# aikiriao/SLA

Hardware: AMD Instinct MI355X
Metric: encode Msamples/s (LPC+residual path), verified bit-exact vs the oracle in this run (higher is better)
Workload: dtype f64+int32

## Files before the change

### sla_amd/csrc/kernels/expand.inc

```
#define EXPAND_THREADS 1024
typedef uint32_t ex_u32x4 __attribute__((ext_vector_type(4), aligned(4)));
typedef uint32_t ex_u32x2 __attribute__((ext_vector_type(2), aligned(4)));
#define EXPAND_PER 8
#define EXPAND_TILE (EXPAND_THREADS * EXPAND_PER)
#define EXPAND_MAX_WINDOWS 256
#define EXPAND_MAX_LEN 16384u
__device__ __forceinline__ uint32_t expand_window(const uint32_t* s_wlen, const uint32_t* s_woff, uint32_t num_win, uint32_t len)
{
  for (uint32_t q = 0; q < num_win; q++) { if (s_wlen[q] == len) { return s_woff[q]; } }
  return SLA_HIP_NO_WINDOW;
}

__device__ __forceinline__ bool expand_range_is_zero(const uint64_t* __restrict__ nz, uint32_t from, uint32_t count)
{
  uint64_t pos = from;
  const uint64_t end = (uint64_t)from + count;
  while (pos < end) {
    const uint64_t word = nz[pos >> 6] >> (pos & 63u);
    if (word != 0ull) { pos += (uint64_t)__builtin_ctzll(word); break; }
    pos += 64u - (pos & 63u);
  }
  return pos >= end;
}

__global__ __launch_bounds__(EXPAND_THREADS)
void k_expand_scan(const sla_hip_superframe* __restrict__ sf, uint32_t num_sf, const uint32_t* __restrict__ parts,
                   const uint32_t* __restrict__ nparts, const uint32_t* __restrict__ status, uint32_t nch,
                   const uint32_t* __restrict__ win_len, uint32_t num_win,
                   uint32_t* __restrict__ run, uint32_t* __restrict__ prefix, uint32_t capacity,
                   volatile uint32_t* counts, uint32_t sequence, const uint64_t* __restrict__ nz)
{
  __shared__ uint32_t s_has[EXPAND_MAX_LEN / 32 + 1];
  __shared__ uint32_t s_cb[EXPAND_TILE], s_cl[EXPAND_TILE];
  __shared__ uint32_t s_wb[EXPAND_THREADS / 64], s_wl[EXPAND_THREADS / 64];
  __shared__ uint32_t s_bad;
  const uint32_t t = threadIdx.x, lane = t & 63, wv = t >> 6;
  if (t == 0) { s_bad = (run[2] != 0u || num_win > EXPAND_MAX_WINDOWS) ? 1u : 0u; }
  for (uint32_t i = t; i < EXPAND_MAX_LEN / 32 + 1; i += EXPAND_THREADS) { s_has[i] = 0u; }
  __syncthreads();
  for (uint32_t i = t; i < num_win && i < EXPAND_MAX_WINDOWS; i += EXPAND_THREADS) {
    const uint32_t len = win_len[i];
    if (len != 0u && len <= EXPAND_MAX_LEN) { atomicOr(&s_has[len >> 5], 1u << (len & 31u)); }
  }
  const uint32_t run_b = run[0], run_g = run[1];
  uint32_t base_b = 0, base_l = 0;
  bool bad = false;
  __syncthreads();
  for (uint32_t t0 = 0; t0 < num_sf; t0 += EXPAND_TILE) {
    uint32_t live[EXPAND_PER], np[EXPAND_PER], st[EXPAND_PER], len0[EXPAND_PER];
#pragma unroll
    for (int k = 0; k < EXPAND_PER; k++) {
      const uint32_t i = t0 + (uint32_t)k * EXPAND_THREADS + t;
      live[k] = (i < num_sf) ? sf[i].live : SLA_HIP_NOT_LIVE;
    }
#pragma unroll
    for (int k = 0; k < EXPAND_PER; k++) {
      const bool l = (live[k] != SLA_HIP_NOT_LIVE);
      np[k] = l ? nparts[live[k]] : 0u;
      st[k] = l ? status[live[k]] : 0u;
      len0[k] = l ? parts[(uint64_t)live[k] * PLAN_NODES] : 0u;
    }
#pragma unroll
    for (int k = 0; k < EXPAND_PER; k++) {
      const uint32_t i = t0 + (uint32_t)k * EXPAND_THREADS + t;
      const bool l = (live[k] != SLA_HIP_NOT_LIVE);
      if (l && (st[k] != 0u || np[k] == 0u || np[k] > PLAN_NODES)) { bad = true; np[k] = 0; }
      uint32_t quiet = 0u, at = (l && nz != nullptr) ? sf[i].start : 0u;
      for (uint32_t p = 0; l && p < np[k]; p++) {
        const uint32_t len = (p == 0) ? len0[k] : parts[(uint64_t)live[k] * PLAN_NODES + p];
        if (len == 0u || len > EXPAND_MAX_LEN || ((s_has[len >> 5] >> (len & 31u)) & 1u) == 0u) { bad = true; }
        else if (nz != nullptr) { if (expand_range_is_zero(nz, at, len)) { quiet++; } at += len; }
      }
      s_cb[(uint32_t)k * EXPAND_THREADS + t] = (i < num_sf) ? (l ? np[k] : 1u) : 0u;
      s_cl[(uint32_t)k * EXPAND_THREADS + t] = l ? np[k] - quiet : 0u;
    }
    __syncthreads();
    uint32_t cb[EXPAND_PER], cl[EXPAND_PER], my_b = 0, my_l = 0;
#pragma unroll
    for (int k = 0; k < EXPAND_PER; k++) { cb[k] = s_cb[t * EXPAND_PER + k]; cl[k] = s_cl[t * EXPAND_PER + k]; my_b += cb[k]; my_l += cl[k]; }
    uint32_t inc_b = my_b, inc_l = my_l;
#pragma unroll
    for (int off = 1; off < 64; off <<= 1) {
      const uint32_t ob = (uint32_t)__shfl_up((int)inc_b, off), ol = (uint32_t)__shfl_up((int)inc_l, off);
      if (lane >= (uint32_t)off) { inc_b += ob; inc_l += ol; }
    }
    if (lane == 63) { s_wb[wv] = inc_b; s_wl[wv] = inc_l; }
    __syncthreads();
    uint32_t off_b = run_b + base_b + (inc_b - my_b), off_l = base_l + (inc_l - my_l), tile_b = 0, tile_l = 0;
    for (uint32_t w = 0; w < EXPAND_THREADS / 64; w++) {
      const uint32_t vb = s_wb[w], vl = s_wl[w];
      if (w < wv) { off_b += vb; off_l += vl; }
      tile_b += vb; tile_l += vl;
    }
#pragma unroll
    for (int k = 0; k < EXPAND_PER; k++) {
      const uint32_t i = t0 + t * EXPAND_PER + (uint32_t)k;
      if (i < num_sf) { ex_u32x2 w; w.x = off_b; w.y = off_l; *reinterpret_cast<ex_u32x2*>(prefix + 2 * (uint64_t)i) = w; }
      off_b += cb[k]; off_l += cl[k];
    }
    base_b += tile_b; base_l += tile_l;
    __syncthreads();
  }
  if (bad) { s_bad = 1u; }
  __syncthreads();
  if (t == 0) {
    const bool ok = (s_bad == 0u) && ((uint64_t)run_g + (uint64_t)base_l * nch <= (uint64_t)capacity);
    run[3] = run_g;
    if (ok) { run[0] = run_b + base_b; run[1] = run_g + base_l * nch; } else { run[2] = 1u; }
    counts[0] = ok ? base_b : 0u; counts[1] = ok ? base_l * nch : 0u; counts[2] = ok ? 1u : 0u;
    __threadfence_system();
    counts[3] = sequence;
    __threadfence_system();
  }
}

__global__ __launch_bounds__(256)
void k_expand_write(const sla_hip_superframe* __restrict__ sf, uint32_t num_sf, const uint32_t* __restrict__ parts,
                    const uint32_t* __restrict__ nparts, uint32_t nch, uint32_t int_shift,
                    const uint32_t* __restrict__ win_len, const uint32_t* __restrict__ win_off, uint32_t num_win,
                    const uint32_t* __restrict__ run, const uint32_t* __restrict__ prefix,
                    sla_hip_lpc_group* __restrict__ groups, sla_hip_lpc_cand* __restrict__ cands, sla_hip_acf_job* __restrict__ acf_jobs,
                    const uint64_t* __restrict__ nz)
{
  __shared__ uint32_t s_wlen[EXPAND_MAX_WINDOWS], s_woff[EXPAND_MAX_WINDOWS];
  if (run[2] != 0u) { return; }
  for (uint32_t i = threadIdx.x; i < num_win && i < EXPAND_MAX_WINDOWS; i += blockDim.x) { s_wlen[i] = win_len[i]; s_woff[i] = win_off[i]; }
  __syncthreads();
  const uint32_t i = blockIdx.x * blockDim.x + threadIdx.x;
  if (i >= num_sf) { return; }
  const sla_hip_superframe f = sf[i];
  if (f.live == SLA_HIP_NOT_LIVE) { return; }
  const uint32_t run_g = run[3];
  const uint32_t np = nparts[f.live];
  uint32_t b = prefix[2 * (uint64_t)i], l = prefix[2 * (uint64_t)i + 1], at = f.start;
  for (uint32_t p = 0; p < np; p++, b++) {
    const uint32_t len = parts[(uint64_t)f.live * PLAN_NODES + p];
    if (nz != nullptr && expand_range_is_zero(nz, at, len)) { at += len; continue; }
    const uint32_t woff = expand_window(s_wlen, s_woff, num_win, len);
    for (uint32_t ch = 0; ch < nch; ch++) {
      const uint32_t g = run_g + l * nch + ch;
      static_assert(sizeof(sla_hip_lpc_group) == 40 && sizeof(sla_hip_lpc_cand) == 8 && sizeof(sla_hip_acf_job) == 16, "descriptor layout");
      ex_u32x4 w0, w1; ex_u32x2 w2, wc; ex_u32x4 wa;
      w0.x = at; w0.y = 0u; w0.z = len; w0.w = ch;
      w1.x = woff; w1.y = int_shift; w1.z = g; w1.w = 1u;
      w2.x = b * nch + ch; w2.y = 0u;
      uint32_t* gp = reinterpret_cast<uint32_t*>(groups + g);
      *reinterpret_cast<ex_u32x4*>(gp) = w0; *reinterpret_cast<ex_u32x4*>(gp + 4) = w1; *reinterpret_cast<ex_u32x2*>(gp + 8) = w2;
      wc.x = 0u; wc.y = len;
      *reinterpret_cast<ex_u32x2*>(cands + g) = wc;
      wa.x = at; wa.y = 0u; wa.z = len; wa.w = ch;
      *reinterpret_cast<ex_u32x4*>(acf_jobs + g) = wa;
    }
    at += len; l++;
  }
}
```

### sla_amd/csrc/kernels/launchers.inc

```
static inline unsigned long long* span_of(const sla_hip_launch_extra* x) { return (x != nullptr) ? x->d_span : nullptr; }

static thread_local sla_hip_tuning t_tuning_val;
static thread_local bool t_tuning_set = false;
extern "C" void sla_hip_use_tuning(const sla_hip_tuning* tuning)
{
  if (tuning != nullptr) { t_tuning_val = *tuning; t_tuning_set = true; } else { t_tuning_set = false; }
}
static inline sla_hip_tuning tuning()
{
  sla_hip_tuning t;
  memset(&t, 0, sizeof(t));
  if (t_tuning_set) { t = t_tuning_val; }
  if (!(t.plan_margin >= PLAN_MARGIN)) { t.plan_margin = 0.0; }
  return t;
}

static hipError_t ensure_dynamic_lds(const void* fn, size_t bytes)
{
  static struct { const void* fn; int dev; size_t bytes; } seen[64];
  static int nseen = 0;
  static pthread_mutex_t mu = PTHREAD_MUTEX_INITIALIZER;
  int dev = 0;
  (void)hipGetDevice(&dev);
  pthread_mutex_lock(&mu);
// ... 411 lines not shown
extern "C" int sla_hip_launch_expand_masked(const sla_hip_superframe* d_superframes, uint32_t num_superframes,
                                     const uint32_t* d_parts, const uint32_t* d_num_parts, const uint32_t* d_status,
                                     uint32_t num_channels, uint32_t int_shift,
                                     const uint32_t* d_win_len, const uint32_t* d_win_off, uint32_t num_windows,
                                     uint32_t* d_run, uint32_t* d_prefix, sla_hip_lpc_group* d_groups, sla_hip_lpc_cand* d_cands,
                                     sla_hip_acf_job* d_acf_jobs, uint32_t group_capacity,
                                     uint32_t* counts, uint32_t sequence, const uint64_t* d_nonzero_mask, sla_hip_stream_t stream);

extern "C" int sla_hip_launch_expand(const sla_hip_superframe* d_superframes, uint32_t num_superframes,
                                     const uint32_t* d_parts, const uint32_t* d_num_parts, const uint32_t* d_status,
                                     uint32_t num_channels, uint32_t int_shift,
                                     const uint32_t* d_win_len, const uint32_t* d_win_off, uint32_t num_windows,
                                     uint32_t* d_run, uint32_t* d_prefix, sla_hip_lpc_group* d_groups, sla_hip_lpc_cand* d_cands,
                                     sla_hip_acf_job* d_acf_jobs, uint32_t group_capacity,
                                     uint32_t* counts, uint32_t sequence, sla_hip_stream_t stream)
{
  return sla_hip_launch_expand_masked(d_superframes, num_superframes, d_parts, d_num_parts, d_status, num_channels, int_shift, d_win_len,
                                      d_win_off, num_windows, d_run, d_prefix, d_groups, d_cands, d_acf_jobs, group_capacity, counts, sequence,
                                      nullptr, stream);
}

extern "C" int sla_hip_launch_expand_masked(const sla_hip_superframe* d_superframes, uint32_t num_superframes,
                                     const uint32_t* d_parts, const uint32_t* d_num_parts, const uint32_t* d_status,
                                     uint32_t num_channels, uint32_t int_shift,
                                     const uint32_t* d_win_len, const uint32_t* d_win_off, uint32_t num_windows,
                                     uint32_t* d_run, uint32_t* d_prefix, sla_hip_lpc_group* d_groups, sla_hip_lpc_cand* d_cands,
                                     sla_hip_acf_job* d_acf_jobs, uint32_t group_capacity,
                                     uint32_t* counts, uint32_t sequence, const uint64_t* d_nonzero_mask, sla_hip_stream_t stream)
{
  if (d_superframes == nullptr || d_parts == nullptr || d_num_parts == nullptr || d_status == nullptr || d_run == nullptr
      || d_prefix == nullptr || d_groups == nullptr || d_cands == nullptr || d_acf_jobs == nullptr || counts == nullptr
      || (num_windows != 0 && (d_win_len == nullptr || d_win_off == nullptr))) { return SLA_APIRESULT_INVALID_ARGUMENT; }
  if (num_channels == 0 || num_channels > 8 || int_shift > 31) { return SLA_APIRESULT_INVALID_ARGUMENT; }
  hipLaunchKernelGGL(k_expand_scan, dim3(1), dim3(EXPAND_THREADS), 0, (hipStream_t)stream, d_superframes, num_superframes, d_parts,
                     d_num_parts, d_status, num_channels, d_win_len, num_windows, d_run, d_prefix, group_capacity,
                     (volatile uint32_t*)counts, sequence, d_nonzero_mask);
  if (num_superframes != 0) {
    hipLaunchKernelGGL(k_expand_write, dim3((num_superframes + 255) / 256), dim3(256), 0, (hipStream_t)stream, d_superframes, num_superframes,
                       d_parts, d_num_parts, num_channels, int_shift, d_win_len, d_win_off, num_windows, d_run, d_prefix, d_groups, d_cands,
                       d_acf_jobs, d_nonzero_mask);
  }
  return hip_rc(hipGetLastError());
}

extern "C" int sla_hip_launch_lattice(const int32_t* d_pcm, uint64_t plane_stride, uint32_t mid_side, uint32_t order,
                                      const sla_hip_lattice_chunk* d_chunks, uint32_t num_chunks,
                                      const int32_t* d_kint, int32_t* d_residual, sla_hip_stream_t stream)
{
  if (d_pcm == nullptr || d_chunks == nullptr || d_kint == nullptr || d_residual == nullptr) { return SLA_APIRESULT_INVALID_ARGUMENT; }
  if (order < 1 || order > 255 || (order + LAT_T - 1) / LAT_T >= 32) { return SLA_APIRESULT_INVALID_ARGUMENT; }
  if (num_chunks == 0) { return 0; }
  hipLaunchKernelGGL(k_lattice, dim3((num_chunks + 3) / 4), dim3(256), 0, (hipStream_t)stream, d_pcm, plane_stride,
                     mid_side, order, d_chunks, num_chunks, d_kint, d_residual, (unsigned long long*)nullptr, tuning().lattice_plain ? 2u : 0u);
  return hip_rc(hipGetLastError());
}

extern "C" int sla_hip_launch_lattice_groups_x(const int32_t* d_pcm, uint64_t plane_stride, uint32_t mid_side, uint32_t order,
                                             const sla_hip_lpc_group* d_groups, uint32_t num_groups, uint32_t max_window,
                                             const int32_t* d_kint, int32_t* d_residual, sla_hip_stream_t stream, const sla_hip_launch_extra* extra)
{
  if (d_pcm == nullptr || d_groups == nullptr || d_kint == nullptr || d_residual == nullptr) { return SLA_APIRESULT_INVALID_ARGUMENT; }
  if (order < 1 || order > 255 || (order + LAT_T - 1) / LAT_T >= 32 || max_window == 0) { return SLA_APIRESULT_INVALID_ARGUMENT; }
  if (num_groups == 0) { return 0; }
  const uint32_t per = (SLA_WAVE - (order + LAT_T - 1) / LAT_T) * LAT_T;
  const uint32_t cpg = (max_window + per - 1) / per;
  const uint64_t waves = (uint64_t)num_groups * cpg;
  if (waves > 0x7FFFFFFFull) { return SLA_APIRESULT_EXCEED_HANDLE_CAPACITY; }
  hipLaunchKernelGGL(k_lattice_groups, dim3((uint32_t)((waves + 3) / 4)), dim3(256), 0, (hipStream_t)stream, d_pcm, plane_stride,
                     mid_side, order, d_groups, num_groups, cpg, d_kint, d_residual, span_of(extra), tuning().lattice_plain ? 2u : 0u);
// ... 277 lines not shown
```

### sla_amd/csrc/sla_encoder.c

```c
#define _GNU_SOURCE
#include "sla_internal.h"
#include "SLADecoder.h"

#include <math.h>
#include <pthread.h>
#include <sched.h>
#include <stdio.h>
#include <stdlib.h>
#include <string.h>
#include <time.h>
#include <unistd.h>

#define STATUS_WAVE_FORMAT   (1u << 0)
#define STATUS_ENCODE_PARAM  (1u << 1)
#define MAX_ANALYSIS_WINDOW  16384u

typedef struct { void* ptr; size_t cap; } devbuf_t;
typedef struct { void* ptr; size_t cap; } pinbuf_t;
typedef struct { void* ptr; size_t cap; } hostbuf_t;

typedef struct {
  uint32_t start, nsmpl, type, bytes;
} blk_t;

// ... 44 lines not shown
  int      device_expand;
  int      expand_silence;
  uint32_t silence_runs;
  devbuf_t d_zruns, d_zscratch; pinbuf_t h_zruns;
  slai_silence sil;
  uint32_t sil_stat[4];
  uint32_t expand_seq;
  uint32_t expanded_chunks;
  int      table_cache, tab_valid;
  uint32_t tab_key[10], tab_cnt[12];
  void*    tab_sf; void* tab_shapes;
  uint32_t winmap_entries;
  uint32_t table_hits;
  int      spec_valid; uint32_t spec_or;
  uint32_t spec_misses;
  uint32_t blocks_exact;
  sla_hip_tuning tune;
  uint32_t host_planned;
  uint32_t fallback_groups;
  uint32_t tail_launches;
  slai_fft_plan* fft;
  uint32_t threads;
  struct slai_pool* pool;

  devbuf_t d_pcm, d_res1, d_res2, d_or, d_nz, d_groups, d_cands, d_lpc_out, d_code, d_kint, d_rshift,
           d_winpool, d_chunks, d_jobs, d_fold, d_acf_jobs, d_acf, d_acf_scratch, d_twiddle, d_bgroups, d_bcands, d_blk_out, d_kk, d_pk_jobs, d_pk_blocks, d_pk_hdr, d_image,
           d_xgroups, d_tile_sums, d_fgroups, d_parts, d_nparts, d_pstatus, d_spans, d_cert_flag, d_fb_list, d_fb_count,
           d_sframes, d_winmap, d_run, d_expref, d_fast_twiddle, d_ltm_eps, d_ltm_list;
  int twiddle_ready;
  pinbuf_t h_nz, h_groups, h_cands, h_lpc_out, h_code, h_kint, h_rshift, h_chunks, h_jobs, h_fold, h_res, h_pcm, h_acf_jobs, h_acf,
           h_bgroups, h_bcands, h_blk_out, h_pk_jobs, h_pk_blocks, h_pk_hdr, h_xgroups, h_fgroups, h_parts, h_nparts, h_pstatus, h_cert_flag,
           h_sframes, h_winmap, h_counts;
  devbuf_t d_rice; pinbuf_t h_rice;
  hostbuf_t w_job_blk, w_job_ch, w_job_grp, w_grp_of_slot, w_parts, w_nparts, w_status;
  uint32_t* h_or;
  size_t nz_ones_cap; uint64_t nz_ones_words;
  pinbuf_t h_stage[2]; devbuf_t d_stage[2]; hipEvent_t ev_stage[2];
  hipEvent_t ev_prep;
  int      groups_valid;
  hipEvent_t ev_pack[4];

  double*   win_host; size_t win_count, win_cap;
  uint32_t* win_len; uint32_t* win_off; uint32_t win_entries, win_entries_cap;
  SLAWindowFunctionType win_type; int win_dirty;

  int32_t* user_res1; int32_t* user_res2; uint64_t user_stride;

  uint32_t file_or_word;
  int      skip_prepass;

  uint32_t nsegs; const uint32_t* seg_start; const uint32_t* seg_len;
  uint32_t batch_lshift, batch_or;
  devbuf_t d_tile_or; pinbuf_t h_tile_or;
  devbuf_t d_binfo; pinbuf_t h_binfo;
  devbuf_t d_ingest; pinbuf_t h_ingest;
  hipEvent_t ev_order;
  int      batch_silence;
  int      mask_absent;
  uint32_t* tab_segs; uint32_t tab_nsegs;

  int      stream_mode;
  uint32_t stream_piece;
  uint32_t stream_lanes;
  uint32_t batch_lanes;
  pthread_mutex_t* upload_gate;
  double   batch_stamp[4];
// ... 1630 lines not shown
  for (j = 0; j < a->njobs; j++) {
    if (e->device_ltm) {
      const sla_hip_tail_job* jb = (const sla_hip_tail_job*)e->h_jobs.ptr + j;
      blkch_t* bc = &e->bc[(size_t)a->job_blk[j] * C + a->job_ch[j]];
      uint32_t t;
      if (e->blk[a->job_blk[j]].type != SLAI_BLK_COMPRESS) { continue; }
      bc->pitch = jb->pitch;
      for (t = 0; t < SLAI_MAX_TAPS; t++) { bc->ltm_q[t] = jb->ltm_coef[t]; }
    }
    {
    const uint64_t mean = fold[j] / e->blk[a->job_blk[j]].nsmpl;
    const uint32_t init = (uint32_t)(mean > 1 ? mean : 1);
    const uint32_t kept = (uint32_t)((((uint64_t)(uint32_t)(init << 8)) + 128u) >> 8);
    e->bc[(size_t)a->job_blk[j] * C + a->job_ch[j]].rice_init = kept ? kept : 1u;
    }
  }
}

typedef struct { struct SLAEncoder* e; const actx_t* a; } home_ctx_t;

static void jobs_home_one(void* vctx, uint32_t j)
{
  const home_ctx_t* c = (const home_ctx_t*)vctx;
  struct SLAEncoder* e = c->e;
  const uint32_t b = c->a->job_blk[j];
  const sla_hip_tail_job* jb = (const sla_hip_tail_job*)e->h_jobs.ptr + j;
  blkch_t* bc = &e->bc[(size_t)b * e->wave_format.num_channels + c->a->job_ch[j]];
  uint32_t t;
  if (e->blk[b].type != SLAI_BLK_COMPRESS) { return; }
  bc->pitch = jb->pitch;
  for (t = 0; t < SLAI_MAX_TAPS; t++) { bc->ltm_q[t] = jb->ltm_coef[t]; }
}

static void rice_home_one(void* vctx, uint32_t j)
{
  const home_ctx_t* c = (const home_ctx_t*)vctx;
  struct SLAEncoder* e = c->e;
  const uint32_t b = c->a->job_blk[j];
  if (e->blk[b].type != SLAI_BLK_COMPRESS) { return; }
  e->bc[(size_t)b * e->wave_format.num_channels + c->a->job_ch[j]].rice_init = ((const uint32_t*)e->h_rice.ptr)[j];
}

static int wait_counts(volatile const uint32_t* hc, uint32_t seq, hipEvent_t done)
{
  uint32_t spins = 0;
  for (;;) {
    if (hc[3] == seq) { __sync_synchronize(); return 0; }
    if ((++spins & 1023u) == 0) {
      const hipError_t q = hipEventQuery(done);
      if (q == hipSuccess) { __sync_synchronize(); return (hc[3] == seq) ? 0 : SLA_APIRESULT_NG; }
      if (q != hipErrorNotReady) { return SLA_APIRESULT_NG; }
    }
    __asm__ volatile("" ::: "memory");
  }
}

static float ev_ms(hipEvent_t s, hipEvent_t t) { float ms = 0.f; return (hipEventElapsedTime(&ms, s, t) == hipSuccess) ? ms : 0.f; }

static int launch_searches(struct SLAEncoder* e, actx_t* a, int preset_blocks, int trace, double t_begin)
{
  const uint32_t C = e->wave_format.num_channels;
  uint32_t c, i, want_chunks;
  int rc = 0;
  e->expand_seq += 1; if (e->expand_seq == 0) { e->expand_seq = 1; }
  memset(a->ck, 0, sizeof(a->ck));
  a->prelaunched = 0;
  a->clear_in_kernel = (!preset_blocks && a->exact);
  if (dev_reserve(&e->d_spans, sizeof(unsigned long long) * SPAN_AREA_ULLS) != 0
      || (!a->clear_in_kernel && hipMemsetAsync(e->d_spans.ptr, 0, sizeof(unsigned long long) * SPAN_AREA_ULLS, e->stream) != hipSuccess)
      || (preset_blocks && hipStreamSynchronize(e->stream) != hipSuccess)) { return SLA_APIRESULT_NG; }
  TRACE("reserved", 0);

  want_chunks = e->chunks;
// ... 44 lines not shown
        if (hipMemsetAsync(e->d_spans.ptr, 0, sizeof(unsigned long long) * SPAN_AREA_ULLS, e->stream) != hipSuccess
            || (a->expand && hipMemsetAsync(e->d_run.ptr, 0, 16, e->stream) != hipSuccess)) { rc = SLA_APIRESULT_NG; }
      }
    }
    if (a->clear_in_kernel) {
      a->clear_ptr[0] = (uint32_t*)e->d_spans.ptr; a->clear_words[0] = SPAN_AREA_ULLS * 2;
      a->clear_ptr[1] = (uint32_t*)e->d_or.ptr + 2; a->clear_words[1] = 1;
      a->clear_ptr[2] = a->expand ? (uint32_t*)e->d_run.ptr : NULL; a->clear_words[2] = 4;
    } else if (hipMemsetAsync((uint32_t*)e->d_or.ptr + 2, 0, sizeof(uint32_t), e->stream) != hipSuccess) { rc = SLA_APIRESULT_NG; }
    for (c = 0; c < a->nchunks && rc == 0; c++) { rc = search_launch(e, a, c); }
    TRACE("search launched", a->nchunks);
  } else {
    a->ck[0].blk_lo = 0; a->ck[0].blk_hi = e->num_blocks;
  }
  return rc;
}


static int run_pipeline(struct SLAEncoder* e, int preset_blocks)
{
  const int trace = e->trace;
  const double t_begin = now_ms();
  const uint32_t C = e->wave_format.num_channels;
  actx_t a;
  uint32_t c, i;
  double t_host = 0.0, t0;
  int rc = 0, tail_queued = 0;
  memset(&a, 0, sizeof(a));
  a.ev = e->ev + 2;

  e->fallback_groups = 0; e->host_planned = 0; e->blocks_exact = 0; e->cert_broken = 0; e->audit_ok = 0; e->audit_bad = 0;
  e->expanded_chunks = 0;
  e->image_valid = 0;
  memset(e->ltm_stat, 0, sizeof(e->ltm_stat));
  e->ltm_cert_now = (e->ltm_cert && e->device_ltm && sla_hip_ltm_cert_supported(slai_fft_plan_size(e->fft)));
  e->cert_now = (e->block_cert && !(e->fuse_lattice && e->encode_param.parcor_order <= 64) && !e->tune.lpc_blocks_chains
                 && sla_hip_search_exact_lags(e->encode_param.parcor_order) != 0);
  a.trace = trace; a.t_begin = t_begin;
  a.fast_rice = (!preset_blocks && e->device_ltm && e->single_tail);
  if (!preset_blocks) {
    e->num_blocks = 0;
    if ((rc = pipeline_prepare(e, &a)) != 0) { actx_free(&a); return rc; }
  } else {
    extern uint32_t sla_hip_lattice_chunk_samples(uint32_t order);
    const uint32_t cs = sla_hip_lattice_chunk_samples(e->encode_param.parcor_order);
    uint32_t woff;
    a.blocks_bound = e->num_blocks;
    for (i = 0; i < e->num_blocks; i++) {
      a.lchunks_bound += C * (e->blk[i].nsmpl / cs + 2);
      if (e->blk[i].type != SLAI_BLK_SILENT && (rc = window_offset(e, e->blk[i].nsmpl, &woff)) != 0) { actx_free(&a); return rc; }
    }
    if ((rc = pin_reserve(&e->h_cands, 64)) != 0 || (rc = pin_reserve(&e->h_groups, 64)) != 0) { actx_free(&a); return rc; }
  }
  {
    const size_t nslots = (size_t)a.blocks_bound * C + 1;
    const size_t nsf1 = (size_t)a.nsf + 1;
    if (host_reserve(&e->w_job_blk, sizeof(uint32_t) * nslots) != 0 || host_reserve(&e->w_job_ch, sizeof(uint32_t) * nslots) != 0
        || host_reserve(&e->w_job_grp, sizeof(uint32_t) * nslots) != 0 || host_reserve(&e->w_grp_of_slot, sizeof(uint32_t) * nslots) != 0
        || host_reserve(&e->w_parts, sizeof(uint32_t) * nsf1 * SLAI_MAX_NODES) != 0
        || host_reserve(&e->w_nparts, sizeof(uint32_t) * nsf1) != 0 || host_reserve(&e->w_status, sizeof(int) * nsf1) != 0) {
      actx_free(&a); return SLA_APIRESULT_NG;
    }
    a.job_blk = (uint32_t*)e->w_job_blk.ptr; a.job_ch = (uint32_t*)e->w_job_ch.ptr; a.job_grp = (uint32_t*)e->w_job_grp.ptr;
    a.grp_of_slot = (uint32_t*)e->w_grp_of_slot.ptr; a.parts = (uint32_t*)e->w_parts.ptr;
    a.nparts = (uint32_t*)e->w_nparts.ptr; a.status = (int*)e->w_status.ptr;
    memset(a.nparts, 0, sizeof(uint32_t) * nsf1);
// ... 110 lines not shown
  memset(e->kernel_ms, 0, sizeof(e->kernel_ms));
  if (rc == 0) {
    const unsigned long long* sp = sp_host;
    int rate_khz = e->wall_clock_khz;
    if (rate_khz <= 0) {
      rate_khz = 100000;
      (void)hipDeviceGetAttribute(&rate_khz, hipDeviceAttributeWallClockRate, e->device);
      if (rate_khz <= 0) { rate_khz = 100000; }
      e->wall_clock_khz = rate_khz;
    }
    if (copied && e->ltm_cert_now) {
      const uint32_t* lc = (const uint32_t*)(sp + SPAN_ULLS);
      for (c = 0; c < a.nchunks; c++) {
        e->ltm_stat[0] += a.ck[c].bg_hi - a.ck[c].bg_lo; e->ltm_stat[2] += lc[4 * c + 1];
        e->ltm_stat[3] += lc[4 * c + 2]; e->ltm_stat[4] += lc[4 * c + 3];
      }
      e->ltm_stat[1] = e->ltm_stat[0] - e->ltm_stat[2];
      e->audit_ok += e->ltm_stat[3]; e->audit_bad += e->ltm_stat[4];
      if (e->ltm_stat[4] != 0) { e->cert_broken = 1; rc = SLA_APIRESULT_NG; }
    }
    if (copied) {
      for (c = 0; c < a.nchunks; c++) {
        for (i = 0; i < 4; i++) {
          const unsigned long long st = ~sp[(c * 4 + i) * 2], en = sp[(c * 4 + i) * 2 + 1];
          if (en != 0 && en > st) { e->kernel_ms[i] += (float)((double)(en - st) / (double)rate_khz); }
        }
      }
    }
  }
  }
  TRACE("all streams idle", 0);
  if (rc == 0) {
    if (a.fast_rice) {
      home_ctx_t hc;
      hc.e = e; hc.a = &a;
      parallel_for(e->pool, a.njobs, rice_home_one, &hc);
    } else {
      finish_rice(e, &a);
    }
    e->timing[0] = preset_blocks ? 0.f : ev_ms(e->ev[0], e->ev[1]);
    e->timing[5] = (float)t_host;
    for (c = 0; c < a.nchunks; c++) {
      hipEvent_t* ev = a.ev + (size_t)c * EV_PER_CHUNK;
      if (!preset_blocks) { e->timing[1] += ev_ms(ev[EV_SEARCH_S], ev[EV_SEARCH_E]); }
      e->timing[2] += ev_ms(ev[EV_LPCB_S], ev[EV_LPCB_E]);
      e->timing[3] += ev_ms(ev[EV_LPCB_E], ev[EV_LAT_E]);
      e->timing[8] += ev_ms(ev[EV_ACF_S], ev[EV_ACF_E]);
      if (!e->single_tail || c == a.nchunks - 1) { e->timing[4] += ev_ms(ev[EV_TAIL_S], ev[EV_TAIL_E]); }
    }
    e->timing[9] = (float)a.nchunks;
    e->tail_launches = (e->single_tail) ? 1u : a.nchunks;
    e->timing[10] = (float)e->fallback_groups;
    e->timing[11] = (float)a.exact;
  }
  TRACE("Rice parameters stored", 0);
  actx_free(&a);
  TRACE("returning", 0);
  return rc;
}

static int enter(struct SLAEncoder* e)
{
  int cur = -1;
  if (hipGetDevice(&cur) != hipSuccess || cur != e->device) { HIPCHK(hipSetDevice(e->device)); }
  sla_hip_use_tuning(&e->tune);
  return 0;
}

int sla_hip_encoder_set_option(struct SLAEncoder* e, const char* name, double value)
// ... 267 lines not shown
int sla_hip_last_timing(const struct SLAEncoder* e, float* timing_ms)
{
  if (e == NULL || timing_ms == NULL) { return SLA_APIRESULT_INVALID_ARGUMENT; }
  memcpy(timing_ms, e->timing, sizeof(e->timing));
  return 0;
}


typedef struct {
  struct SLAEncoder* e;
  const int32_t* res;
  const int32_t* const* pcm;
  uint8_t** bufs; uint32_t* sizes;
} pack_ctx_t;

static void pack_one(void* vctx, uint32_t b)
{
  pack_ctx_t* c = (pack_ctx_t*)vctx;
  struct SLAEncoder* e = c->e;
  const uint32_t C = e->wave_format.num_channels, O1 = e->encode_param.parcor_order + 1;
  const blk_t* k = &e->blk[b];
  slai_block_params bp;
  uint32_t rshift[SLAI_MAX_CHANNELS], pitch[SLAI_MAX_CHANNELS], rice[SLAI_MAX_CHANNELS], ch, s;
  int32_t ltm[SLAI_MAX_CHANNELS * SLAI_MAX_TAPS];
  int32_t* raw[SLAI_MAX_CHANNELS] = {0};
  uint32_t cap = 64 + C * (8 + 2 * O1 + 16);
  uint8_t* buf;
  memset(&bp, 0, sizeof(bp));
  bp.num_samples = k->nsmpl; bp.type = k->type; bp.num_channels = C; bp.order = O1 - 1;
  bp.ntaps = e->encode_param.longterm_order; bp.bps = e->wave_format.bit_per_sample; bp.lshift = e->lshift;
  bp.mid_side = (e->encode_param.ch_process_method == SLA_CHPROCESSMETHOD_STEREO_MS);
  for (ch = 0; ch < C; ch++) {
    const blkch_t* bc = &e->bc[(size_t)b * C + ch];
    rshift[ch] = bc->rshift; pitch[ch] = bc->pitch; rice[ch] = bc->rice_init;
    memcpy(&ltm[ch * SLAI_MAX_TAPS], bc->ltm_q, sizeof(int32_t) * SLAI_MAX_TAPS);
  }
  bp.code = e->code + (size_t)b * C * O1; bp.rshift = rshift; bp.pitch = pitch; bp.ltm_q = ltm; bp.rice_init = rice;
  if (k->type == SLAI_BLK_COMPRESS) {
    for (ch = 0; ch < C; ch++) { bp.res[ch] = c->res + (size_t)ch * e->num_samples + k->start; }
    cap += 8 * C * k->nsmpl;
  } else if (k->type == SLAI_BLK_RAW) {
    const uint32_t shift = 32 - bp.bps + e->lshift;
    for (ch = 0; ch < C; ch++) { raw[ch] = (int32_t*)malloc(sizeof(int32_t) * k->nsmpl); bp.res[ch] = raw[ch]; }
    for (s = 0; s < k->nsmpl; s++) {
      if (bp.mid_side) {
        const int32_t l = c->pcm[0][k->start + s] >> shift, r = c->pcm[1][k->start + s] >> shift;
        raw[0][s] = (int32_t)((uint32_t)l + (uint32_t)r) >> 1;
        raw[1][s] = (int32_t)((uint32_t)l - (uint32_t)r);
      } else {
        for (ch = 0; ch < C; ch++) { raw[ch][s] = c->pcm[ch][k->start + s] >> shift; }
      }
    }
    cap += 8 * C * k->nsmpl;
  }
  for (;;) {
    buf = (uint8_t*)malloc(cap);
    if (buf == NULL) { c->sizes[b] = 0; break; }
    c->sizes[b] = slai_pack_block(&bp, buf, cap);
    if (c->sizes[b] != 0 || cap > (1u << 30)) { break; }
    free(buf); buf = NULL;
    cap *= 4;
  }
  c->bufs[b] = buf;
  for (ch = 0; ch < C; ch++) { free(raw[ch]); }
}

static int pack_impl(struct SLAEncoder* e, const int32_t* const* host_pcm, uint8_t* data, uint32_t data_size, uint32_t* output_size)
// ... 67 lines not shown
  uint8_t* data; uint32_t data_size;
  uint32_t out_size; int result;
  uint32_t num_blocks, max_block, max_bps;
  uint64_t img_off;
  int bare;
  int (*place)(void* ctx, uint32_t out_size, uint8_t** data, uint32_t* data_size);
  void* place_ctx;
} pack_seg_t;

static int download_bytes(struct SLAEncoder* e, uint8_t* dst, const uint8_t* d_src, size_t bytes);

typedef struct {
  struct SLAEncoder* e; sla_hip_pack_block* pb; sla_hip_rice_job* jobs; uint8_t* hdr; const uint32_t* job_of; int bad;
  int what;
} pack_hdr_ctx_t;

static void pack_hdr_one(void* vctx, uint32_t b)
{
  pack_hdr_ctx_t* c = (pack_hdr_ctx_t*)vctx;
  struct SLAEncoder* e = c->e;
  const uint32_t C = e->wave_format.num_channels, O1 = e->encode_param.parcor_order + 1;
  const blk_t* k = &e->blk[b];
  sla_hip_pack_block* pb = &c->pb[b];
  slai_block_params bp;
  uint32_t rshift[SLAI_MAX_CHANNELS], pitch[SLAI_MAX_CHANNELS], rice[SLAI_MAX_CHANNELS], ch;
  int32_t ltm[SLAI_MAX_CHANNELS * SLAI_MAX_TAPS];
  uint8_t tmp[16];
  memset(&bp, 0, sizeof(bp));
  bp.num_samples = k->nsmpl; bp.type = k->type; bp.num_channels = C; bp.order = O1 - 1;
  bp.ntaps = e->encode_param.longterm_order; bp.bps = e->wave_format.bit_per_sample; bp.lshift = e->lshift;
  bp.mid_side = (e->encode_param.ch_process_method == SLA_CHPROCESSMETHOD_STEREO_MS);
  for (ch = 0; ch < C; ch++) {
    const blkch_t* bc = &e->bc[(size_t)b * C + ch];
    rshift[ch] = bc->rshift; pitch[ch] = bc->pitch; rice[ch] = bc->rice_init;
    memcpy(&ltm[ch * SLAI_MAX_TAPS], bc->ltm_q, sizeof(int32_t) * SLAI_MAX_TAPS);
  }
  bp.code = e->code + (size_t)b * C * O1; bp.rshift = rshift; bp.pitch = pitch; bp.ltm_q = ltm; bp.rice_init = rice;
  if (c->what == 1) {
    pb->blk_off = k->start; pb->num_samples = k->nsmpl; pb->type = k->type;
    pb->raw_bits = bp.bps - e->lshift;
    if (k->type == SLAI_BLK_COMPRESS) {
      slai_coding_mode(rice, C, pb->golomb_m);
      for (ch = 0; ch < C; ch++) {
        sla_hip_rice_job* j = &c->jobs[c->job_of[b] + ch];
        j->blk_off = k->start; j->blk_len = k->nsmpl; j->channel = ch; j->rice_init = rice[ch]; j->golomb_m = pb->golomb_m[ch];
      }
    }
    return;
  }
  if (pb->header_bytes >= 16) {
    if (slai_pack_header(&bp, c->hdr + pb->header_off, pb->header_bytes) != pb->header_bytes) { c->bad = 1; return; }
  } else {
    const uint32_t got = slai_pack_header(&bp, tmp, sizeof(tmp));
    if (got != pb->header_bytes) { c->bad = 1; return; }
    memcpy(c->hdr + pb->header_off, tmp, got);
  }
}

typedef struct {
  uint32_t nvb, nsegs;
  uint64_t compared;
  size_t   rep_off;
} verify_run_t;

static void verify_clear(struct SLAEncoder* e) { memset(e->ver, 0, sizeof(e->ver)); e->ver_ran = 0; }

static void verify_add(struct SLAEncoder* e, const uint64_t v[5])
// ... 1437 lines not shown
  return RES1(e);
}

int sla_hip_bind_residual_planes(struct SLAEncoder* e, int32_t* d_lattice, int32_t* d_final, uint64_t plane_stride)
{
  if (e == NULL || ((d_lattice == NULL) != (d_final == NULL))) { return SLA_APIRESULT_INVALID_ARGUMENT; }
  e->user_res1 = d_lattice; e->user_res2 = d_final; e->user_stride = plane_stride;
  e->analysed = 0;
  return 0;
}

int sla_hip_get_trace(struct SLAEncoder* e, sla_hip_trace* tr)
{
  uint32_t C, O1, b, ch, t;
  if (e == NULL || tr == NULL) { return SLA_APIRESULT_INVALID_ARGUMENT; }
  if (!e->analysed) { return SLA_APIRESULT_PARAMETER_NOT_SET; }
  RCCHK(enter(e));
  C = e->wave_format.num_channels; O1 = e->encode_param.parcor_order + 1;
  if (tr->max_blocks < e->num_blocks || tr->order_stride < O1 || tr->sample_stride < e->num_samples
      || (tr->ltm_stride < e->encode_param.longterm_order)) { return SLA_APIRESULT_INSUFFICIENT_BUFFER_SIZE; }
  tr->num_blocks = e->num_blocks; tr->offset_lshift = e->lshift;
  for (b = 0; b < e->num_blocks; b++) {
    tr->blk_start[b] = e->blk[b].start; tr->blk_nsmpl[b] = e->blk[b].nsmpl;
    tr->blk_type[b] = e->blk[b].type; tr->blk_bytes[b] = e->blk[b].bytes;
    for (ch = 0; ch < C; ch++) {
      const size_t slot = (size_t)b * C + ch;
      const blkch_t* bc = &e->bc[slot];
      if (e->blk[b].type != SLAI_BLK_COMPRESS) { tr->rshift[slot] = 0; tr->pitch[slot] = 0; tr->rice_init[slot] = 0; continue; }
      for (t = 0; t < O1; t++) {
        tr->parcor[slot * tr->order_stride + t] = e->parcor[slot * O1 + t];
        tr->code[slot * tr->order_stride + t] = e->code[slot * O1 + t];
        tr->kint[slot * tr->order_stride + t] = e->kint[slot * O1 + t];
      }
      tr->rshift[slot] = bc->rshift; tr->pitch[slot] = bc->pitch; tr->rice_init[slot] = bc->rice_init;
      if (tr->parcor_exact != NULL) { tr->parcor_exact[slot] = e->parcor_exact[slot]; }
      for (t = 0; t < e->encode_param.longterm_order; t++) { tr->ltm_coef[slot * tr->ltm_stride + t] = bc->ltm_q[t]; }
    }
  }
  for (ch = 0; ch < C && e->num_samples > 0; ch++) {
    if (tr->res_lattice != NULL && RES1(e) != NULL) {
      HIPCHK(hipMemcpy(tr->res_lattice + (size_t)ch * tr->sample_stride, RES1(e) + (size_t)ch * e->stride,
                       sizeof(int32_t) * e->num_samples, hipMemcpyDeviceToHost));
    }
    if (tr->res_final != NULL && RES2(e) != NULL) {
      HIPCHK(hipMemcpy(tr->res_final + (size_t)ch * tr->sample_stride, RES2(e) + (size_t)ch * e->stride,
                       sizeof(int32_t) * e->num_samples, hipMemcpyDeviceToHost));
    }
  }
  return 0;
}
```

Before: 50190.

## Parallelize expand scan across tiles and read rice params lazily from host buffer

The single-block expand scan, which walked all superframe tiles serially, is split into a multi-block per-tile scan, a one-wave kernel that scans the tile totals, and a write kernel that adds tile base and local offset. Separately, the host no longer copies fast-rice results into per-block structs with a parallel_for; consumers read them on demand through a slot-to-group map. This removes a serial GPU bottleneck and a host copy pass, at the cost of an extra kernel launch and an indirection on each rice lookup.

```diff
diff --git a/sla_amd/csrc/kernels/expand.inc b/sla_amd/csrc/kernels/expand.inc
--- a/sla_amd/csrc/kernels/expand.inc
+++ b/sla_amd/csrc/kernels/expand.inc
@@ -5,6 +5,7 @@
 #define EXPAND_TILE (EXPAND_THREADS * EXPAND_PER)
 #define EXPAND_MAX_WINDOWS 256
 #define EXPAND_MAX_LEN 16384u
+#define EXPAND_TILE_BAD 0xFFFFFFFFu
 __device__ __forceinline__ uint32_t expand_window(const uint32_t* s_wlen, const uint32_t* s_woff, uint32_t num_win, uint32_t len)
 {
   for (uint32_t q = 0; q < num_win; q++) { if (s_wlen[q] == len) { return s_woff[q]; } }
@@ -24,87 +25,111 @@
 }
 
 __global__ __launch_bounds__(EXPAND_THREADS)
-void k_expand_scan(const sla_hip_superframe* __restrict__ sf, uint32_t num_sf, const uint32_t* __restrict__ parts,
-                   const uint32_t* __restrict__ nparts, const uint32_t* __restrict__ status, uint32_t nch,
-                   const uint32_t* __restrict__ win_len, uint32_t num_win,
-                   uint32_t* __restrict__ run, uint32_t* __restrict__ prefix, uint32_t capacity,
-                   volatile uint32_t* counts, uint32_t sequence, const uint64_t* __restrict__ nz)
+void k_expand_tiles(const sla_hip_superframe* __restrict__ sf, uint32_t num_sf, const uint32_t* __restrict__ parts,
+                    const uint32_t* __restrict__ nparts, const uint32_t* __restrict__ status,
+                    const uint32_t* __restrict__ win_len, uint32_t num_win,
+                    uint32_t* __restrict__ prefix, const uint64_t* __restrict__ nz)
 {
   __shared__ uint32_t s_has[EXPAND_MAX_LEN / 32 + 1];
   __shared__ uint32_t s_cb[EXPAND_TILE], s_cl[EXPAND_TILE];
   __shared__ uint32_t s_wb[EXPAND_THREADS / 64], s_wl[EXPAND_THREADS / 64];
-  __shared__ uint32_t s_bad;
   const uint32_t t = threadIdx.x, lane = t & 63, wv = t >> 6;
-  if (t == 0) { s_bad = (run[2] != 0u || num_win > EXPAND_MAX_WINDOWS) ? 1u : 0u; }
+  const uint32_t t0 = blockIdx.x * EXPAND_TILE;
   for (uint32_t i = t; i < EXPAND_MAX_LEN / 32 + 1; i += EXPAND_THREADS) { s_has[i] = 0u; }
   __syncthreads();
   for (uint32_t i = t; i < num_win && i < EXPAND_MAX_WINDOWS; i += EXPAND_THREADS) {
     const uint32_t len = win_len[i];
     if (len != 0u && len <= EXPAND_MAX_LEN) { atomicOr(&s_has[len >> 5], 1u << (len & 31u)); }
   }
-  const uint32_t run_b = run[0], run_g = run[1];
-  uint32_t base_b = 0, base_l = 0;
   bool bad = false;
   __syncthreads();
-  for (uint32_t t0 = 0; t0 < num_sf; t0 += EXPAND_TILE) {
-    uint32_t live[EXPAND_PER], np[EXPAND_PER], st[EXPAND_PER], len0[EXPAND_PER];
+  uint32_t live[EXPAND_PER], np[EXPAND_PER], st[EXPAND_PER], len0[EXPAND_PER];
 #pragma unroll
-    for (int k = 0; k < EXPAND_PER; k++) {
-      const uint32_t i = t0 + (uint32_t)k * EXPAND_THREADS + t;
-      live[k] = (i < num_sf) ? sf[i].live : SLA_HIP_NOT_LIVE;
+  for (int k = 0; k < EXPAND_PER; k++) {
+    const uint32_t i = t0 + (uint32_t)k * EXPAND_THREADS + t;
+    live[k] = (i < num_sf) ? sf[i].live : SLA_HIP_NOT_LIVE;
+  }
+#pragma unroll
+  for (int k = 0; k < EXPAND_PER; k++) {
+    const bool l = (live[k] != SLA_HIP_NOT_LIVE);
+    np[k] = l ? nparts[live[k]] : 0u;
+    st[k] = l ? status[live[k]] : 0u;
+    len0[k] = l ? parts[(uint64_t)live[k] * PLAN_NODES] : 0u;
+  }
+#pragma unroll
+  for (int k = 0; k < EXPAND_PER; k++) {
+    const uint32_t i = t0 + (uint32_t)k * EXPAND_THREADS + t;
+    const bool l = (live[k] != SLA_HIP_NOT_LIVE);
+    if (l && (st[k] != 0u || np[k] == 0u || np[k] > PLAN_NODES)) { bad = true; np[k] = 0; }
+    uint32_t quiet = 0u, at = (l && nz != nullptr) ? sf[i].start : 0u;
+    for (uint32_t p = 0; l && p < np[k]; p++) {
+      const uint32_t len = (p == 0) ? len0[k] : parts[(uint64_t)live[k] * PLAN_NODES + p];
+      if (len == 0u || len > EXPAND_MAX_LEN || ((s_has[len >> 5] >> (len & 31u)) & 1u) == 0u) { bad = true; }
+      else if (nz != nullptr) { if (expand_range_is_zero(nz, at, len)) { quiet++; } at += len; }
     }
+    s_cb[(uint32_t)k * EXPAND_THREADS + t] = (i < num_sf) ? (l ? np[k] : 1u) : 0u;
+    s_cl[(uint32_t)k * EXPAND_THREADS + t] = l ? np[k] - quiet : 0u;
+  }
+  const bool tile_bad = (__syncthreads_or(bad ? 1 : 0) != 0);
+  uint32_t cb[EXPAND_PER], cl[EXPAND_PER], my_b = 0, my_l = 0;
 #pragma unroll
-    for (int k = 0; k < EXPAND_PER; k++) {
-      const bool l = (live[k] != SLA_HIP_NOT_LIVE);
-      np[k] = l ? nparts[live[k]] : 0u;
-      st[k] = l ? status[live[k]] : 0u;
-      len0[k] = l ? parts[(uint64_t)live[k] * PLAN_NODES] : 0u;
+  for (int k = 0; k < EXPAND_PER; k++) { cb[k] = s_cb[t * EXPAND_PER + k]; cl[k] = s_cl[t * EXPAND_PER + k]; my_b += cb[k]; my_l += cl[k]; }
+  uint32_t inc_b = my_b, inc_l = my_l;
+#pragma unroll
+  for (int off = 1; off < 64; off <<= 1) {
+    const uint32_t ob = (uint32_t)__shfl_up((int)inc_b, off), ol = (uint32_t)__shfl_up((int)inc_l, off);
+    if (lane >= (uint32_t)off) { inc_b += ob; inc_l += ol; }
+  }
+  if (lane == 63) { s_wb[wv] = inc_b; s_wl[wv] = inc_l; }
+  __syncthreads();
+  uint32_t off_b = inc_b - my_b, off_l = inc_l - my_l, tile_b = 0, tile_l = 0;
+  for (uint32_t w = 0; w < EXPAND_THREADS / 64; w++) {
+    const uint32_t vb = s_wb[w], vl = s_wl[w];
+    if (w < wv) { off_b += vb; off_l += vl; }
+    tile_b += vb; tile_l += vl;
+  }
+#pragma unroll
+  for (int k = 0; k < EXPAND_PER; k++) {
+    const uint32_t i = t0 + t * EXPAND_PER + (uint32_t)k;
+    if (i < num_sf) {
+      ex_u32x2 w; w.x = off_b; w.y = off_l;
+      if (t == 0 && k == 0) { w.x = tile_bad ? EXPAND_TILE_BAD : tile_b; w.y = tile_l; }
+      *reinterpret_cast<ex_u32x2*>(prefix + 2 * (uint64_t)i) = w;
     }
-#pragma unroll
-    for (int k = 0; k < EXPAND_PER; k++) {
-      const uint32_t i = t0 + (uint32_t)k * EXPAND_THREADS + t;
-      const bool l = (live[k] != SLA_HIP_NOT_LIVE);
-      if (l && (st[k] != 0u || np[k] == 0u || np[k] > PLAN_NODES)) { bad = true; np[k] = 0; }
-      uint32_t quiet = 0u, at = (l && nz != nullptr) ? sf[i].start : 0u;
-      for (uint32_t p = 0; l && p < np[k]; p++) {
-        const uint32_t len = (p == 0) ? len0[k] : parts[(uint64_t)live[k] * PLAN_NODES + p];
-        if (len == 0u || len > EXPAND_MAX_LEN || ((s_has[len >> 5] >> (len & 31u)) & 1u) == 0u) { bad = true; }
-        else if (nz != nullptr) { if (expand_range_is_zero(nz, at, len)) { quiet++; } at += len; }
-      }
-      s_cb[(uint32_t)k * EXPAND_THREADS + t] = (i < num_sf) ? (l ? np[k] : 1u) : 0u;
-      s_cl[(uint32_t)k * EXPAND_THREADS + t] = l ? np[k] - quiet : 0u;
-    }
-    __syncthreads();
-    uint32_t cb[EXPAND_PER], cl[EXPAND_PER], my_b = 0, my_l = 0;
-#pragma unroll
-    for (int k = 0; k < EXPAND_PER; k++) { cb[k] = s_cb[t * EXPAND_PER + k]; cl[k] = s_cl[t * EXPAND_PER + k]; my_b += cb[k]; my_l += cl[k]; }
-    uint32_t inc_b = my_b, inc_l = my_l;
+    off_b += cb[k]; off_l += cl[k];
+  }
+}
+
+__global__ __launch_bounds__(64)
+void k_expand_sum(uint32_t num_sf, uint32_t nch, uint32_t num_win, uint32_t* __restrict__ run, uint32_t* __restrict__ prefix,
+                  uint32_t capacity, volatile uint32_t* counts, uint32_t sequence)
+{
+  const uint32_t lane = threadIdx.x;
+  const uint32_t ntiles = (num_sf + EXPAND_TILE - 1) / EXPAND_TILE;
+  const uint32_t run_b = run[0], run_g = run[1];
+  bool bad = (run[2] != 0u || num_win > EXPAND_MAX_WINDOWS);
+  uint32_t base_b = 0, base_l = 0;
+  for (uint32_t q0 = 0; q0 < ntiles; q0 += 64) {
+    const uint32_t q = q0 + lane;
+    uint32_t* slot = prefix + 2 * (uint64_t)q * EXPAND_TILE;
+    ex_u32x2 w; w.x = 0u; w.y = 0u;
+    if (q < ntiles) { w = *reinterpret_cast<const ex_u32x2*>(slot); }
+    if (w.x == EXPAND_TILE_BAD) { bad = true; w.x = 0u; w.y = 0u; }
+    uint32_t inc_b = w.x, inc_l = w.y;
 #pragma unroll
     for (int off = 1; off < 64; off <<= 1) {
       const uint32_t ob = (uint32_t)__shfl_up((int)inc_b, off), ol = (uint32_t)__shfl_up((int)inc_l, off);
       if (lane >= (uint32_t)off) { inc_b += ob; inc_l += ol; }
     }
-    if (lane == 63) { s_wb[wv] = inc_b; s_wl[wv] = inc_l; }
-    __syncthreads();
-    uint32_t off_b = run_b + base_b + (inc_b - my_b), off_l = base_l + (inc_l - my_l), tile_b = 0, tile_l = 0;
-    for (uint32_t w = 0; w < EXPAND_THREADS / 64; w++) {
-      const uint32_t vb = s_wb[w], vl = s_wl[w];
-      if (w < wv) { off_b += vb; off_l += vl; }
-      tile_b += vb; tile_l += vl;
+    if (q < ntiles) {
+      ex_u32x2 o; o.x = run_b + base_b + (inc_b - w.x); o.y = base_l + (inc_l - w.y);
+      *reinterpret_cast<ex_u32x2*>(slot) = o;
     }
-#pragma unroll
-    for (int k = 0; k < EXPAND_PER; k++) {
-      const uint32_t i = t0 + t * EXPAND_PER + (uint32_t)k;
-      if (i < num_sf) { ex_u32x2 w; w.x = off_b; w.y = off_l; *reinterpret_cast<ex_u32x2*>(prefix + 2 * (uint64_t)i) = w; }
-      off_b += cb[k]; off_l += cl[k];
-    }
-    base_b += tile_b; base_l += tile_l;
-    __syncthreads();
+    base_b += (uint32_t)__shfl((int)inc_b, 63); base_l += (uint32_t)__shfl((int)inc_l, 63);
   }
-  if (bad) { s_bad = 1u; }
-  __syncthreads();
-  if (t == 0) {
-    const bool ok = (s_bad == 0u) && ((uint64_t)run_g + (uint64_t)base_l * nch <= (uint64_t)capacity);
+  bad = (__any(bad ? 1 : 0) != 0);
+  if (lane == 0) {
+    const bool ok = !bad && ((uint64_t)run_g + (uint64_t)base_l * nch <= (uint64_t)capacity);
     run[3] = run_g;
     if (ok) { run[0] = run_b + base_b; run[1] = run_g + base_l * nch; } else { run[2] = 1u; }
     counts[0] = ok ? base_b : 0u; counts[1] = ok ? base_l * nch : 0u; counts[2] = ok ? 1u : 0u;
@@ -132,7 +157,9 @@
   if (f.live == SLA_HIP_NOT_LIVE) { return; }
   const uint32_t run_g = run[3];
   const uint32_t np = nparts[f.live];
-  uint32_t b = prefix[2 * (uint64_t)i], l = prefix[2 * (uint64_t)i + 1], at = f.start;
+  const uint32_t i0 = i - (i % EXPAND_TILE);
+  uint32_t b = prefix[2 * (uint64_t)i0], l = prefix[2 * (uint64_t)i0 + 1], at = f.start;
+  if (i != i0) { b += prefix[2 * (uint64_t)i]; l += prefix[2 * (uint64_t)i + 1]; }
   for (uint32_t p = 0; p < np; p++, b++) {
     const uint32_t len = parts[(uint64_t)f.live * PLAN_NODES + p];
     if (nz != nullptr && expand_range_is_zero(nz, at, len)) { at += len; continue; }
diff --git a/sla_amd/csrc/kernels/launchers.inc b/sla_amd/csrc/kernels/launchers.inc
--- a/sla_amd/csrc/kernels/launchers.inc
+++ b/sla_amd/csrc/kernels/launchers.inc
@@ -467,9 +467,12 @@
       || d_prefix == nullptr || d_groups == nullptr || d_cands == nullptr || d_acf_jobs == nullptr || counts == nullptr
       || (num_windows != 0 && (d_win_len == nullptr || d_win_off == nullptr))) { return SLA_APIRESULT_INVALID_ARGUMENT; }
   if (num_channels == 0 || num_channels > 8 || int_shift > 31) { return SLA_APIRESULT_INVALID_ARGUMENT; }
-  hipLaunchKernelGGL(k_expand_scan, dim3(1), dim3(EXPAND_THREADS), 0, (hipStream_t)stream, d_superframes, num_superframes, d_parts,
-                     d_num_parts, d_status, num_channels, d_win_len, num_windows, d_run, d_prefix, group_capacity,
-                     (volatile uint32_t*)counts, sequence, d_nonzero_mask);
+  if (num_superframes != 0) {
+    hipLaunchKernelGGL(k_expand_tiles, dim3((num_superframes + EXPAND_TILE - 1) / EXPAND_TILE), dim3(EXPAND_THREADS), 0, (hipStream_t)stream,
+                       d_superframes, num_superframes, d_parts, d_num_parts, d_status, d_win_len, num_windows, d_prefix, d_nonzero_mask);
+  }
+  hipLaunchKernelGGL(k_expand_sum, dim3(1), dim3(64), 0, (hipStream_t)stream, num_superframes, num_channels, num_windows, d_run, d_prefix,
+                     group_capacity, (volatile uint32_t*)counts, sequence);
   if (num_superframes != 0) {
     hipLaunchKernelGGL(k_expand_write, dim3((num_superframes + 255) / 256), dim3(256), 0, (hipStream_t)stream, d_superframes, num_superframes,
                        d_parts, d_num_parts, num_channels, int_shift, d_win_len, d_win_off, num_windows, d_run, d_prefix, d_groups, d_cands,
diff --git a/sla_amd/csrc/sla_encoder.c b/sla_amd/csrc/sla_encoder.c
--- a/sla_amd/csrc/sla_encoder.c
+++ b/sla_amd/csrc/sla_encoder.c
@@ -100,6 +100,7 @@
            h_bgroups, h_bcands, h_blk_out, h_pk_jobs, h_pk_blocks, h_pk_hdr, h_xgroups, h_fgroups, h_parts, h_nparts, h_pstatus, h_cert_flag,
            h_sframes, h_winmap, h_counts;
   devbuf_t d_rice; pinbuf_t h_rice;
+  int rice_in_h;
   hostbuf_t w_job_blk, w_job_ch, w_job_grp, w_grp_of_slot, w_parts, w_nparts, w_status;
   uint32_t* h_or;
   size_t nz_ones_cap; uint64_t nz_ones_words;
@@ -1796,13 +1797,13 @@
   for (t = 0; t < SLAI_MAX_TAPS; t++) { bc->ltm_q[t] = jb->ltm_coef[t]; }
 }
 
-static void rice_home_one(void* vctx, uint32_t j)
-{
-  const home_ctx_t* c = (const home_ctx_t*)vctx;
-  struct SLAEncoder* e = c->e;
-  const uint32_t b = c->a->job_blk[j];
-  if (e->blk[b].type != SLAI_BLK_COMPRESS) { return; }
-  e->bc[(size_t)b * e->wave_format.num_channels + c->a->job_ch[j]].rice_init = ((const uint32_t*)e->h_rice.ptr)[j];
+static uint32_t rice_word(const struct SLAEncoder* e, uint32_t b, uint32_t ch)
+{
+  const size_t slot = (size_t)b * e->wave_format.num_channels + ch;
+  if (e->rice_in_h && e->blk[b].type == SLAI_BLK_COMPRESS) {
+    return ((const uint32_t*)e->h_rice.ptr)[((const uint32_t*)e->w_grp_of_slot.ptr)[slot]];
+  }
+  return e->bc[slot].rice_init;
 }
 
 static int wait_counts(volatile const uint32_t* hc, uint32_t seq, hipEvent_t done)
@@ -1913,6 +1914,7 @@
   e->fallback_groups = 0; e->host_planned = 0; e->blocks_exact = 0; e->cert_broken = 0; e->audit_ok = 0; e->audit_bad = 0;
   e->expanded_chunks = 0;
   e->image_valid = 0;
+  e->rice_in_h = 0;
   memset(e->ltm_stat, 0, sizeof(e->ltm_stat));
   e->ltm_cert_now = (e->ltm_cert && e->device_ltm && sla_hip_ltm_cert_supported(slai_fft_plan_size(e->fft)));
   e->cert_now = (e->block_cert && !(e->fuse_lattice && e->encode_param.parcor_order <= 64) && !e->tune.lpc_blocks_chains
@@ -2089,9 +2091,7 @@
   TRACE("all streams idle", 0);
   if (rc == 0) {
     if (a.fast_rice) {
-      home_ctx_t hc;
-      hc.e = e; hc.a = &a;
-      parallel_for(e->pool, a.njobs, rice_home_one, &hc);
+      e->rice_in_h = 1;
     } else {
       finish_rice(e, &a);
     }
@@ -2425,7 +2425,7 @@
   bp.mid_side = (e->encode_param.ch_process_method == SLA_CHPROCESSMETHOD_STEREO_MS);
   for (ch = 0; ch < C; ch++) {
     const blkch_t* bc = &e->bc[(size_t)b * C + ch];
-    rshift[ch] = bc->rshift; pitch[ch] = bc->pitch; rice[ch] = bc->rice_init;
+    rshift[ch] = bc->rshift; pitch[ch] = bc->pitch; rice[ch] = rice_word(e, b, ch);
     memcpy(&ltm[ch * SLAI_MAX_TAPS], bc->ltm_q, sizeof(int32_t) * SLAI_MAX_TAPS);
   }
   bp.code = e->code + (size_t)b * C * O1; bp.rshift = rshift; bp.pitch = pitch; bp.ltm_q = ltm; bp.rice_init = rice;
@@ -2559,7 +2559,7 @@
   bp.mid_side = (e->encode_param.ch_process_method == SLA_CHPROCESSMETHOD_STEREO_MS);
   for (ch = 0; ch < C; ch++) {
     const blkch_t* bc = &e->bc[(size_t)b * C + ch];
-    rshift[ch] = bc->rshift; pitch[ch] = bc->pitch; rice[ch] = bc->rice_init;
+    rshift[ch] = bc->rshift; pitch[ch] = bc->pitch; rice[ch] = rice_word(e, b, ch);
     memcpy(&ltm[ch * SLAI_MAX_TAPS], bc->ltm_q, sizeof(int32_t) * SLAI_MAX_TAPS);
   }
   bp.code = e->code + (size_t)b * C * O1; bp.rshift = rshift; bp.pitch = pitch; bp.ltm_q = ltm; bp.rice_init = rice;
@@ -4063,7 +4063,7 @@
         tr->code[slot * tr->order_stride + t] = e->code[slot * O1 + t];
         tr->kint[slot * tr->order_stride + t] = e->kint[slot * O1 + t];
       }
-      tr->rshift[slot] = bc->rshift; tr->pitch[slot] = bc->pitch; tr->rice_init[slot] = bc->rice_init;
+      tr->rshift[slot] = bc->rshift; tr->pitch[slot] = bc->pitch; tr->rice_init[slot] = rice_word(e, b, ch);
       if (tr->parcor_exact != NULL) { tr->parcor_exact[slot] = e->parcor_exact[slot]; }
       for (t = 0; t < e->encode_param.longterm_order; t++) { tr->ltm_coef[slot * tr->ltm_stride + t] = bc->ltm_q[t]; }
     }
```

Result: slower. 49420 (-1.5%).
